# AlwinEsch/pvr.rtl.radiofm

Measured on AMD Instinct MI355X. Metric: IQ MS/s demodulated (whole node) + achieved HBM GB/s on FIR stage, higher is better.
Workload: dtype f32

## Files before the change

pvr.rtl.radiofm_amd/csrc/fmd_k_serial.hip.h:

```cpp
#pragma once

#include "fmd_k_common.hip.h"

namespace fmd
{


#ifndef FMD_DS
#define FMD_DS 32
#endif
constexpr int DS = FMD_DS;
static_assert(DS == 32 || DS == 16, "chunk size");
typedef float fmd_v4f __attribute__((ext_vector_type(4)));
constexpr int STAGE_RS = 65;
constexpr unsigned FM_UNROLL = 4;

template <int NG, bool EXCL, bool MIX = true>
__global__ __launch_bounds__(128 * NG) void k_demod_serial(
    const float2* __restrict__ demod, unsigned Mstride, unsigned M, unsigned C, unsigned CP,
    DemodConsts k, ChannelState st, float2* __restrict__ br, unsigned Hbb,
    float2* __restrict__ mix, unsigned Hmix, const double* __restrict__ sctab_g, FmdSincosTab sct,
    unsigned stereo_q, long long* __restrict__ wg_probe, float osc_after_re, float osc_after_im)
{
  const long long probe_r0 = wg_probe ? (long long)__builtin_amdgcn_s_memrealtime() : 0;
  const long long probe_c0 = wg_probe ? (long long)__builtin_readcyclecounter() : 0;
  __shared__ float chunk_all[NG][2][DS][64];
  __shared__ float2 stage_all[NG][2][DS][STAGE_RS];
  constexpr unsigned SCTAB_N = FMD_SINCOS_P256_SIZE;
  __shared__ __attribute__((aligned(1024))) double sctab[2 * SCTAB_N];
  __shared__ __attribute__((aligned(512))) float atab[FMD_ATAN_TAB_FLOATS];
  constexpr bool PAIRSYNC = NG > 1;
  __shared__ unsigned done_all[NG][2];
  if (threadIdx.x < 2 * NG)
    (&done_all[0][0])[threadIdx.x] = 0;
  __builtin_amdgcn_s_setprio(3);
  if (EXCL)
    asm volatile("" ::: "v255", "a255");
  for (unsigned i = threadIdx.x; i < 2 * SCTAB_N; i += 128 * NG)
    sctab[i] = sctab_g[i];
  if (threadIdx.x == 0)
    fmd_atan_table_fill(atab);
  const unsigned lane = threadIdx.x & 63u;
  const unsigned wave = threadIdx.x >> 6;
  const unsigned role = wave & 1u;
  const unsigned grp = wave >> 1;
  float (*chunk)[DS][64] = chunk_all[grp];
  float2 (*stage)[DS][STAGE_RS] = stage_all[grp];
  const unsigned done_fm = (unsigned)(size_t)&done_all[grp][0];
  const unsigned done_2nd = (unsigned)(size_t)&done_all[grp][1];
  double m16 = -1.0 / 6.0;
  asm volatile("" : "+v"(m16));
  const unsigned c0 = (blockIdx.x * NG + grp) * 64 + lane;
  const bool active = c0 < C;
  const unsigned c = active ? c0 : C - 1;
  const unsigned nchunks = (M + DS - 1) / DS;
  const float2* __restrict__ row = demod + (size_t)c * Mstride;
  for (unsigned u = role; u < DS; u += 2)
    stage[0][u][lane] = row[min(u, M - 1)];
  __syncthreads();

  if (role == 0)
  {
    float nco_phase = st.F(F_NCO_PHASE)[c], nco_incr = st.F(F_NCO_INCR)[c];
    __builtin_amdgcn_s_waitcnt(0);
    for (unsigned j = 0; j <= nchunks; j++)
    {
      if (PAIRSYNC)
      {
        if (j == nchunks)
          break;
        lds_wait_ge(done_2nd, j, st.spin_limit, st.err);
      }
      if (j < nchunks)
      {
        const unsigned m0 = j * DS;
        const unsigned cnt = min((unsigned)DS, M - m0);
        auto fm_sample = [&](unsigned u) -> uint32_t {
          const float2 sin_ = stage[j & 1][u][lane];
          const float sre = sin_.x, sim = sin_.y;
          float sn, cs;
          fmd_sincos_p256_finish(fmd_sincos_p256_lookup_lds(nco_phase, sctab), m16, &sn, &cs);
          const fmd_v2f dd = fmd_pk_add_cross((fmd_v2f){sre, sim} * cs, (fmd_v2f){sre, sim} * sn);
          const float dre = dd.x, dim = dd.y;
          uint32_t lit;
          const float err = -fmd_atan2f_tab_core(dim, dre, atab, &lit);
          const fmd_v2f ba = (fmd_v2f){k.pll_beta, k.pll_alpha} * err;
          nco_incr += ba.x;
          nco_incr = fminf(fmaxf(nco_incr, k.nco_ll), k.nco_hl);
          nco_phase += nco_incr + ba.y;
          {
            const uint32_t pb = fmd_f2u(nco_phase);
            uint32_t khi = (~pb & 0x80000000u) | 0x401921fbu;
            khi = pb < 0x40c90fdbu ? 0u : khi;
            const uint64_t kb = ((uint64_t)khi << 32) | 0x54442d18u;
            double off;
            memcpy(&off, &kb, 8);
            nco_phase = (float)((double)nco_phase + off);
          }
          chunk[j & 1][u][lane] = nco_incr;
          return lit;
        };
        auto fm_sample_literal = [&](unsigned u) {
          const float2 sin_ = stage[j & 1][u][lane];
          float sn, cs;
          fmd_sincos_p256k(nco_phase, sctab, m16, &sn, &cs);
          const fmd_v2f dd = fmd_pk_add_cross((fmd_v2f){sin_.x, sin_.y} * cs, (fmd_v2f){sin_.x, sin_.y} * sn);
          const float e2 = -fmd_atan2f(dd.y, dd.x);
          float in2 = nco_incr + k.pll_beta * e2;
          in2 = (in2 < k.nco_ll) ? k.nco_ll : in2;
          in2 = (in2 > k.nco_hl) ? k.nco_hl : in2;
          float ph2 = nco_phase + (in2 + k.pll_alpha * e2);
          const double pd2 = (double)ph2;
          if (pd2 >= FMD_K_2PI)
            ph2 = (float)fmod(pd2, FMD_K_2PI);
          while (ph2 < 0)
            ph2 = (float)((double)ph2 + FMD_K_2PI);
          nco_incr = in2;
          nco_phase = ph2;
          chunk[j & 1][u][lane] = nco_incr;
        };
#ifdef FMD_DBG_NO_FM
        if (true)
        {
          for (unsigned u = 0; u < cnt; u++)
            chunk[j & 1][u][lane] = nco_incr;
        }
        else
#endif
        if (cnt == (unsigned)DS)
        {
#pragma unroll 1
          for (unsigned u = 0; u < (unsigned)DS; u += FM_UNROLL)
          {
            const float phase_g = nco_phase, incr_g = nco_incr;
            uint32_t worst = 0;
#pragma unroll
            for (unsigned v = 0; v < FM_UNROLL; v++)
              worst = max(worst, fm_sample(u + v));
            if (__builtin_expect(FMD_ANY_LANE(worst >= FMD_ATAN_RARE_LIMIT), 0))
            {
              nco_phase = phase_g;
              nco_incr = incr_g;
#pragma unroll 1
              for (unsigned v = 0; v < FM_UNROLL; v++)
                fm_sample_literal(u + v);
            }
          }
        }
        else
        {
#pragma unroll 1
          for (unsigned u = 0; u < cnt; u++)
          {
            const float phase_g = nco_phase, incr_g = nco_incr;
            if (__builtin_expect(FMD_ANY_LANE(fm_sample(u) >= FMD_ATAN_RARE_LIMIT), 0))
            {
              nco_phase = phase_g;
              nco_incr = incr_g;
              fm_sample_literal(u);
            }
          }
        }
      }
      if (PAIRSYNC)
        lds_publish(done_fm, j + 1);
      else
        lds_barrier();
    }
    if (active)
    {
      st.F(F_NCO_PHASE)[c] = nco_phase;
      st.F(F_NCO_INCR)[c] = nco_incr;
    }
  }
  else
  {
    float p_i1 = st.F(F_P_I1)[c], p_i2 = st.F(F_P_I2)[c], p_q1 = st.F(F_P_Q1)[c], p_q2 = st.F(F_P_Q2)[c];
    float p_x1 = st.F(F_P_X1)[c], p_freq = st.F(F_P_FREQ)[c], p_phase = st.F(F_P_PHASE)[c];
    float p_level = 1000.0f;
    float o_re = st.F(F_OSC_RE)[c], o_im = st.F(F_OSC_IM)[c];
    float dc = st.F(F_DC_OFF)[c];
    __builtin_amdgcn_s_waitcnt(0);
    FmdSincosP256 p_sc = fmd_sincos_p256_lookup_lds(p_phase, sctab);
    float vsum = 0.0f, vsumsq = 0.0f;
    char* __restrict__ br_rows = reinterpret_cast<char*>(br + (size_t)Hbb * CP);
    char* __restrict__ mix_rows = reinterpret_cast<char*>(mix + (size_t)Hmix * CP);
    unsigned row_off = c * (unsigned)sizeof(float2);
    const unsigned row_step = CP * (unsigned)sizeof(float2);
    constexpr unsigned CO_LPR = DS / 2;
    constexpr unsigned CO_RPI = 64 / CO_LPR;
    const unsigned co_row = lane / CO_LPR, co_col = lane % CO_LPR;
    unsigned co_off[DS / 2];
#pragma unroll
    for (unsigned i = 0; i < DS / 2; i++)
      co_off[i] = min((blockIdx.x * NG + grp) * 64 + CO_RPI * i + co_row, C - 1) *
                      (Mstride * (unsigned)sizeof(float2)) +
                  co_col * 16u;
    for (unsigned j = 0; j <= nchunks; j++)
    {
      const unsigned pf0 = (j + 1) * DS;
      const bool staging = (j + 1) < nchunks;
      fmd_v4f pre_c[DS / 2];
      if (staging)
      {
        const float2* sb = demod + pf0;
#pragma unroll
        for (unsigned i = 0; i < DS / 2; i += 4)
          asm volatile("global_load_dwordx4 %0, %4, %8\n\t"
                       "global_load_dwordx4 %1, %5, %8\n\t"
                       "global_load_dwordx4 %2, %6, %8\n\t"
                       "global_load_dwordx4 %3, %7, %8"
                       : "=&v"(pre_c[i]), "=&v"(pre_c[i + 1]), "=&v"(pre_c[i + 2]), "=&v"(pre_c[i + 3])
                       : "v"(co_off[i]), "v"(co_off[i + 1]), "v"(co_off[i + 2]), "v"(co_off[i + 3]), "s"(sb)
                       : "memory");
      }
      unsigned stores_behind = 0;
      if (PAIRSYNC && j >= 1)
        lds_wait_ge(done_fm, j, st.spin_limit, st.err);
      if (j >= 1)
      {
        const unsigned m0 = (j - 1) * DS;
        const unsigned cnt = min((unsigned)DS, M - m0);
        float pinc_next = chunk[(j - 1) & 1][0][lane];
        auto second_sample = [&](unsigned u) {
            const float pinc = 2 * pinc_next;
            pinc_next = chunk[(j - 1) & 1][min(u + 1, (unsigned)DS - 1)][lane];
            dc = (float)((1 - 0.0001) * (double)dc + 0.0001 * (double)pinc);
            const float v = (pinc - dc) * k.demod_gain;
            vsum += v;
            vsumsq += v * v;
            float ps, pc;
            fmd_sincos_p256_finish(p_sc, m16, &ps, &pc);
            const float tone = 2 * ps * pc;
            float ph_i = ps * v;
            float ph_q = pc * v;
            ph_i = k.p_b0 * ph_i - k.p_a1 * p_i1 - k.p_a2 * p_i2;
            ph_q = k.p_b0 * ph_q - k.p_a1 * p_q1 - k.p_a2 * p_q2;
            p_i2 = p_i1;
            p_i1 = ph_i;
            p_q2 = p_q1;
            p_q1 = ph_q;
            const float ratio = ph_q / ph_i;
            const float sgn = (ph_q > 0) ? 1.0f : -1.0f;
            const float perr = (ph_i > fabsf(ph_q)) ? ratio : sgn;
            p_level = (ph_i < p_level) ? ph_i : p_level;
            p_freq += k.p_lf_b0 * perr + k.p_lf_b1 * p_x1;
            p_x1 = perr;
            p_freq = fmaxf(k.p_minfreq, fminf(k.p_maxfreq, p_freq));
            p_phase += p_freq;
            {
              const double pd = (double)p_phase;
              const float down = (float)(pd - FMD_K_2PI);
              p_phase = (pd > FMD_K_2PI) ? down : p_phase;
            }
            p_sc = fmd_sincos_p256_lookup_lds(p_phase, sctab);
            __builtin_amdgcn_sched_barrier(0);
            if constexpr (MIX)
            {
            float2 osc;
            osc.x = o_re * k.osc_cos - o_im * k.osc_sin;
            osc.y = o_im * k.osc_cos + o_re * k.osc_sin;
            const float gn = (float)(1.95 - (double)(o_re * o_re + o_im * o_im));
            o_re = gn * osc.x;
            o_im = gn * osc.y;
            const float zero = 0.0f;
#ifdef FMD_DBG_NO_STORES
            vsum += tone * (2 * v) + ((v * osc.x) - (zero * osc.y)) + ((v * osc.y) + (zero * osc.x));
#else
            *reinterpret_cast<float2*>(br_rows + row_off) = make_float2(v, tone * (2 * v));
            *reinterpret_cast<float2*>(mix_rows + row_off) =
                make_float2((v * osc.x) - (zero * osc.y), (v * osc.y) + (zero * osc.x));
#endif
            }
            else
              *reinterpret_cast<float2*>(br_rows + row_off) = make_float2(v, tone * (2 * v));
            row_off += row_step;
        };
#ifdef FMD_DBG_NO_2ND
        if (true)
        {
        }
        else
#endif
        if (cnt == (unsigned)DS)
        {
#pragma unroll 1
          for (unsigned u = 0; u < (unsigned)DS; u += 2)
          {
            second_sample(u);
            second_sample(u + 1);
          }
        }
        else
        {
#pragma unroll 1
          for (unsigned u = 0; u < cnt; u++)
            second_sample(u);
        }
        stores_behind = (MIX ? 2 : 1) * cnt;
      }
      if (staging)
      {
        if (stores_behind >= (MIX ? 2 : 1) * DS)
        {
          if ((MIX ? 2 : 1) * DS == 64)
            asm volatile("s_waitcnt vmcnt(63)" ::: "memory");
          else if ((MIX ? 2 : 1) * DS == 32)
            asm volatile("s_waitcnt vmcnt(31)" ::: "memory");
          else
            asm volatile("s_waitcnt vmcnt(15)" ::: "memory");
        }
        else
          asm volatile("s_waitcnt vmcnt(0)" ::: "memory");
#pragma unroll
        for (unsigned i = 0; i < DS / 2; i++)
        {
          stage[(j + 1) & 1][2 * co_col][CO_RPI * i + co_row] = make_float2(pre_c[i].x, pre_c[i].y);
          stage[(j + 1) & 1][2 * co_col + 1][CO_RPI * i + co_row] = make_float2(pre_c[i].z, pre_c[i].w);
        }
      }
      if (PAIRSYNC)
        lds_publish(done_2nd, j + 1);
      else
        lds_barrier();
    }
    if (active)
    {
      st.F(F_P_I1)[c] = p_i1;
      st.F(F_P_I2)[c] = p_i2;
      st.F(F_P_Q1)[c] = p_q1;
      st.F(F_P_Q2)[c] = p_q2;
      st.F(F_P_X1)[c] = p_x1;
      st.F(F_P_FREQ)[c] = p_freq;
      st.F(F_P_PHASE)[c] = p_phase;
      st.F(F_P_LEVEL)[c] = p_level;
      st.F(F_OSC_RE)[c] = MIX ? o_re : osc_after_re;
      st.F(F_OSC_IM)[c] = MIX ? o_im : osc_after_im;
      st.F(F_DC_OFF)[c] = dc;
      {
        int cnt = st.I(I_P_LOCK_CNT)[c];
        if (2 * p_level > k.p_minsignal)
        {
          if (cnt < k.p_lock_delay)
            cnt += (int)M;
        }
        else
          cnt = 0;
        st.I(I_P_LOCK_CNT)[c] = cnt;
        st.I(I_STEREO)[c] = cnt >= k.p_lock_delay;
        st.I(I_STEREO_Q0 + (int)stereo_q)[c] = cnt >= k.p_lock_delay;
      }
      {
        const float mean = vsum / (float)M;
        const float rms = sqrtf(vsumsq / (float)M);
        st.F(F_BB_MEAN)[c] = 0.95f * st.F(F_BB_MEAN)[c] + 0.05f * mean;
        st.F(F_BB_LEVEL)[c] = 0.95f * st.F(F_BB_LEVEL)[c] + 0.05f * rms;
      }
    }
  }
  if (wg_probe && threadIdx.x == 64)
  {
    wg_probe[3 * blockIdx.x] = probe_r0;
    wg_probe[3 * blockIdx.x + 1] = (long long)__builtin_amdgcn_s_memrealtime();
    const unsigned hw_id = __builtin_amdgcn_s_getreg((31 << 11) | 4);
    const unsigned xcc_id = __builtin_amdgcn_s_getreg((31 << 11) | 20);
    wg_probe[3 * blockIdx.x + 2] = (((long long)__builtin_readcyclecounter() - probe_c0) & 0xffffffffffll) |
                                   ((long long)((hw_id >> 8) & 0xffu) << 40) |
                                   ((long long)(xcc_id & 0xfu) << 48);
  }
}

}
```

pvr.rtl.radiofm_amd/csrc/fmd_math.h:

```cpp
#ifndef FMD_MATH_H
#define FMD_MATH_H

#include <math.h>
#include <stdint.h>
#include <string.h>
#ifndef __cplusplus
#include <stdbool.h>
#endif

#ifdef __HIPCC__
#define FMD_HD __host__ __device__ static inline
#define FMD_HD_NOINLINE __host__ __device__ static __attribute__((noinline))
#else
#define FMD_HD static inline
#define FMD_HD_NOINLINE static __attribute__((noinline))
#endif

#if defined(__clang__)
typedef float fmd_v2f __attribute__((ext_vector_type(2)));
#else
typedef float fmd_v2f __attribute__((vector_size(8)));
#endif

FMD_HD fmd_v2f fmd_pk_add_cross(fmd_v2f a, fmd_v2f b)
{
#if defined(__HIP_DEVICE_COMPILE__)
  fmd_v2f r;
  asm("v_pk_add_f32 %0, %1, %2 op_sel:[0,1] op_sel_hi:[1,0] neg_lo:[0,1]" : "=v"(r) : "v"(a), "v"(b));
  return r;
#else
  fmd_v2f r = {a[0] - b[1], a[1] + b[0]};
  return r;
#endif
}

#define FMD_K_2PI (2.0 * 3.14159265358979323846)
#define FMD_K_PI (3.14159265358979323846)
#define FMD_K_PI2 (FMD_K_PI / 2.0)

#if defined(__HIP_DEVICE_COMPILE__)
#define FMD_ANY_LANE(cond) (__builtin_amdgcn_ballot_w64(cond) != 0)
#else
#define FMD_ANY_LANE(cond) (cond)
#endif

FMD_HD float fmd_div_midrange(float n, float d)
{
#if defined(__HIP_DEVICE_COMPILE__)
  const float r0 = __builtin_amdgcn_rcpf(d);
  const float e0 = __builtin_fmaf(-d, r0, 1.0f);
  const float r1 = __builtin_fmaf(e0, r0, r0);
  const float q0 = n * r1;
  const float e1 = __builtin_fmaf(-d, q0, n);
  const float q1 = __builtin_fmaf(e1, r1, q0);
  const float e2 = __builtin_fmaf(-d, q1, n);
  return __builtin_fmaf(e2, r1, q1);
#else
  return n / d;
#endif
}

FMD_HD uint32_t fmd_f2u(float f)
{
  uint32_t u;
  memcpy(&u, &f, 4);
  return u;
}
FMD_HD float fmd_u2f(uint32_t u)
{
  float f;
  memcpy(&f, &u, 4);
  return f;
}

FMD_HD float fmd_u8_to_f32(unsigned b)
{
  const float f = (float)b;
  const float s = __builtin_fmaf(f, 0x1.01p-7f, -1.0f);
  return __builtin_fmaf(f, 0x1.010102p-23f, s);
}

FMD_HD float fmd_s8_to_f32(int v)
{
  return (float)v * 0x1p-7f;
}
FMD_HD float fmd_s16_to_f32(int v)
{
  return (float)v * 0x1p-15f;
}

FMD_HD float fmd_ciq16_to_f32(int v)
{
  return (float)v * 0x1p-13f;
}

FMD_HD int fmd_f32_to_s16_count(float x, unsigned* clipped)
{
  const float y = x * 32768.0f;
  if (y != y)
    return 0;
  const float r = rintf(y);
  *clipped += (r > 32767.0f) | (r < -32768.0f);
  return (int)fminf(fmaxf(r, -32768.0f), 32767.0f);
}
FMD_HD int fmd_f32_to_s16(float x)
{
  unsigned clipped = 0;
  return fmd_f32_to_s16_count(x, &clipped);
}

FMD_HD int fmd_f32_to_mpx16(float x)
{
  const float y = x * 8192.0f;
  if (y != y)
    return 0;
  return (int)fminf(fmaxf(rintf(y), -32768.0f), 32767.0f);
}

FMD_HD float fmd_atanf(float x)
{
  const float atanhi0 = 4.6364760399e-01f, atanhi1 = 7.8539812565e-01f,
              atanhi2 = 9.8279368877e-01f, atanhi3 = 1.5707962513e+00f;
  const float atanlo0 = 5.0121582440e-09f, atanlo1 = 3.7748947079e-08f,
              atanlo2 = 3.4473217170e-08f, atanlo3 = 7.5497894159e-08f;
  const float aT0 = 3.3333334327e-01f, aT1 = -2.0000000298e-01f, aT2 = 1.4285714924e-01f,
              aT3 = -1.1111110449e-01f, aT4 = 9.0908870101e-02f, aT5 = -7.6918758452e-02f,
              aT6 = 6.6610731184e-02f, aT7 = -5.8335702866e-02f, aT8 = 4.9768779427e-02f,
              aT9 = -3.6531571299e-02f, aT10 = 1.6285819933e-02f;
  const float one = 1.0f;
  float w, s1, s2, z;
  int32_t hx = (int32_t)fmd_f2u(x);
  int32_t ix = hx & 0x7fffffff;
  int id;
  float hi = 0.0f, lo = 0.0f;
  if (ix >= 0x4c000000)
  {
    if (ix > 0x7f800000)
      return x + x;
    if (hx > 0)
      return atanhi3 + atanlo3;
    return -atanhi3 - atanlo3;
  }
  if (ix < 0x3ee00000)
  {
    if (ix < 0x31000000)
      return x;
    id = -1;
  }
  else
  {
    x = fabsf(x);
    if (ix < 0x3f980000)
    {
      if (ix < 0x3f300000)
      {
        id = 0;
        x = (2.0f * x - one) / (2.0f + x);
        hi = atanhi0;
        lo = atanlo0;
      }
      else
      {
        id = 1;
        x = (x - one) / (x + one);
        hi = atanhi1;
        lo = atanlo1;
      }
    }
    else
    {
      if (ix < 0x401c0000)
      {
        id = 2;
        x = (x - 1.5f) / (one + 1.5f * x);
        hi = atanhi2;
        lo = atanlo2;
      }
      else
      {
        id = 3;
        x = -1.0f / x;
        hi = atanhi3;
        lo = atanlo3;
      }
    }
  }
  z = x * x;
  w = z * z;
  s1 = z * (aT0 + w * (aT2 + w * (aT4 + w * (aT6 + w * (aT8 + w * aT10)))));
  s2 = w * (aT1 + w * (aT3 + w * (aT5 + w * (aT7 + w * aT9))));
  if (id < 0)
    return x - x * (s1 + s2);
  z = hi - ((x * (s1 + s2) - lo) - x);
  return (hx < 0) ? -z : z;
}

FMD_HD_NOINLINE float fmd_atan2f(float y, float x)
{
  const float tiny = 1.0e-30f, pi_o_4 = 7.8539818525e-01f, pi_o_2 = 1.5707963705e+00f,
              pi = 3.1415927410e+00f, pi_lo = -8.7422776573e-08f;
  float z;
  int32_t hx = (int32_t)fmd_f2u(x), hy = (int32_t)fmd_f2u(y);
  int32_t ix = hx & 0x7fffffff, iy = hy & 0x7fffffff;
  if ((ix > 0x7f800000) || (iy > 0x7f800000))
    return x + y;
  if (hx == 0x3f800000)
    return fmd_atanf(y);
  int m = ((hy >> 31) & 1) | ((hx >> 30) & 2);
  if (iy == 0)
  {
    switch (m)
    {
      case 0:
      case 1:
        return y;
      case 2:
        return pi + tiny;
      default:
        return -pi - tiny;
    }
  }
  if (ix == 0)
    return (hy < 0) ? -pi_o_2 - tiny : pi_o_2 + tiny;
  if (ix == 0x7f800000)
  {
    if (iy == 0x7f800000)
    {
      switch (m)
      {
        case 0:
          return pi_o_4 + tiny;
        case 1:
          return -pi_o_4 - tiny;
        case 2:
          return 3.0f * pi_o_4 + tiny;
        default:
          return -3.0f * pi_o_4 - tiny;
      }
    }
    else
    {
      switch (m)
      {
        case 0:
          return 0.0f;
        case 1:
          return -0.0f;
        case 2:
          return pi + tiny;
        default:
          return -pi - tiny;
      }
    }
  }
  if (iy == 0x7f800000)
    return (hy < 0) ? -pi_o_2 - tiny : pi_o_2 + tiny;
  int32_t k = (iy - ix) >> 23;
  if (k > 60)
    z = pi_o_2 + 0.5f * pi_lo;
  else if (hx < 0 && k < -60)
    z = 0.0f;
  else
    z = fmd_atanf(fabsf(y / x));
  switch (m)
  {
    case 0:
      return z;
    case 1:
      return fmd_u2f(fmd_f2u(z) ^ 0x80000000u);
    case 2:
      return pi - (z - pi_lo);
    default:
      return (z - pi_lo) - pi;
  }
}

FMD_HD void fmd_sincos_nco(float phase, float* s, float* c)
{
  const double x = (double)phase;
  const double k = __builtin_rint(x * 6.36619772367581382433e-01);
  double r = __builtin_fma(-k, 1.57079632673412561417e+00, x);
  r = __builtin_fma(-k, 6.07710050650619224932e-11, r);
  const double z = r * r;
  double ps = __builtin_fma(z, 1.58969099521155010221e-10, -2.50507602534068634195e-08);
  ps = __builtin_fma(z, ps, 2.75573137070700676789e-06);
  ps = __builtin_fma(z, ps, -1.98412698298579493134e-04);
  ps = __builtin_fma(z, ps, 8.33333333332248946124e-03);
  ps = __builtin_fma(z, ps, -1.66666666666666324348e-01);
  const double sr = __builtin_fma(r * z, ps, r);
  double pc = __builtin_fma(z, -1.13596475577881948265e-11, 2.08757232129817482790e-09);
  pc = __builtin_fma(z, pc, -2.75573143513906633035e-07);
  pc = __builtin_fma(z, pc, 2.48015872894767294178e-05);
  pc = __builtin_fma(z, pc, -1.38888888888741095749e-03);
  pc = __builtin_fma(z, pc, 4.16666666666666019037e-02);
  const double hz = 0.5 * z;
  const double w = 1.0 - hz;
  const double cr = w + (((1.0 - w) - hz) + z * z * pc);
  const int n = (int)k;
  double so = (n & 1) ? cr : sr;
  double co = (n & 1) ? sr : cr;
  so = (n & 2) ? -so : so;
  co = ((n + 1) & 2) ? -co : co;
  *s = (float)so;
  *c = (float)co;
}

#define FMD_ATAN_TAB_FLOATS 40
FMD_HD void fmd_atan_table_fill(float* t)
{
  const float v[5][8] = {
      {1.0f, 0.0f, 0.0f, 1.0f, 0.0f, 0.0f, 0, 0},
      {2.0f, -1.0f, 1.0f, 2.0f, 4.6364760399e-01f, 5.0121582440e-09f, 0, 0},
      {1.0f, -1.0f, 1.0f, 1.0f, 7.8539812565e-01f, 3.7748947079e-08f, 0, 0},
      {1.0f, -1.5f, 1.5f, 1.0f, 9.8279368877e-01f, 3.4473217170e-08f, 0, 0},
      {0.0f, -1.0f, 1.0f, 0.0f, 1.5707962513e+00f, 7.5497894159e-08f, 0, 0}};
  for (int r = 0; r < 5; r++)
    for (int k = 0; k < 8; k++)
      t[r * 8 + k] = v[r][k];
}

#if defined(__HIP_DEVICE_COMPILE__)
FMD_HD unsigned long long fmd_pack2f(float lo, float hi)
{
  return (unsigned long long)fmd_f2u(lo) | ((unsigned long long)fmd_f2u(hi) << 32);
}
#endif

#define FMD_ATAN_RARE_LIMIT (0x4c000000u - 0x31000000u)
FMD_HD float fmd_atan2f_tab_core(float y, float x, const float* tab, uint32_t* rare_measure)
{
  const float aT0 = 3.3333334327e-01f, aT1 = -2.0000000298e-01f, aT2 = 1.4285714924e-01f,
              aT3 = -1.1111110449e-01f, aT4 = 9.0908870101e-02f, aT5 = -7.6918758452e-02f,
              aT6 = 6.6610731184e-02f, aT7 = -5.8335702866e-02f, aT8 = 4.9768779427e-02f,
              aT9 = -3.6531571299e-02f, aT10 = 1.6285819933e-02f;
  const float pi = 3.1415927410e+00f, pi_lo = -8.7422776573e-08f;
  const float q = fabsf(y / x);
  const uint32_t iq = fmd_f2u(q);
  const uint32_t rare_m = iq - 0x31000000u;
  const uint32_t ic = iq;
  const float qc = fmd_u2f(ic);
  const int r = 4 + ((int32_t)(ic - 0x3ee00000u) >> 31) + ((int32_t)(ic - 0x3f300000u) >> 31) +
                ((int32_t)(ic - 0x3f980000u) >> 31) + ((int32_t)(ic - 0x401c0000u) >> 31);
  const float* t = tab + 8 * r;
#if defined(__HIP_DEVICE_COMPILE__)
  const float a2 = (float)__builtin_amdgcn_ubfe(0x02242u, 4u * (unsigned)r, 4u);
  const float c2 = (float)__builtin_amdgcn_ubfe(0x23220u, 4u * (unsigned)r, 4u);
#else
  const float a2 = (float)((0x02242u >> (4u * (unsigned)r)) & 0xfu);
  const float c2 = (float)((0x23220u >> (4u * (unsigned)r)) & 0xfu);
#endif
  const fmd_v2f ac = {a2, c2};
  const fmd_v2f nd = fmd_pk_add_cross(ac * qc, ac);
  const float num = nd[0];
  const float den = nd[1];
  const float xr = fmd_div_midrange(num, den);
  const float z = xr * xr;
  const float w = z * z;
  const fmd_v2f wz = {w, z};
  fmd_v2f hc;
#if defined(__HIP_DEVICE_COMPILE__)
  asm("v_pk_mul_f32 %0, %1, %2 op_sel_hi:[0,1]\n\t"
      "v_pk_add_f32 %0, %0, %3\n\t"
      "v_pk_mul_f32 %0, %0, %1 op_sel_hi:[1,0]\n\t"
      "v_pk_add_f32 %0, %0, %4\n\t"
      "v_pk_mul_f32 %0, %0, %1 op_sel_hi:[1,0]\n\t"
      "v_pk_add_f32 %0, %0, %5\n\t"
      "v_pk_mul_f32 %0, %0, %1 op_sel_hi:[1,0]\n\t"
      "v_pk_add_f32 %0, %0, %6\n\t"
      "v_pk_mul_f32 %0, %0, %1 op_sel_hi:[1,0]\n\t"
      "v_pk_add_f32 %0, %0, %7\n\t"
      "v_pk_mul_f32 %0, %0, %1"
      : "=&v"(hc)
      : "v"(wz), "s"(fmd_pack2f(0.0f, aT10)), "s"(fmd_pack2f(aT9, aT8)), "s"(fmd_pack2f(aT7, aT6)),
        "s"(fmd_pack2f(aT5, aT4)), "s"(fmd_pack2f(aT3, aT2)), "s"(fmd_pack2f(aT1, aT0)));
#else
  hc = (fmd_v2f){0.0f, aT10} * w + (fmd_v2f){aT9, aT8};
  hc = hc * w + (fmd_v2f){aT7, aT6};
  hc = hc * w + (fmd_v2f){aT5, aT4};
  hc = hc * w + (fmd_v2f){aT3, aT2};
  hc = hc * w + (fmd_v2f){aT1, aT0};
  hc = hc * wz;
#endif
  const float p = xr * (hc[1] + hc[0]);
  const float at = t[4] - ((p - t[5]) - xr);
  const float left = pi - (at - pi_lo);
  const float base = ((int32_t)fmd_f2u(x) < 0) ? left : at;
  *rare_measure = rare_m;
  return fmd_u2f(fmd_f2u(base) ^ (fmd_f2u(y) & 0x80000000u));
}

FMD_HD float fmd_atan2f_tab(float y, float x, const float* tab)
{
  uint32_t rare_m;
  float res = fmd_atan2f_tab_core(y, x, tab, &rare_m);
  const bool rare = rare_m >= FMD_ATAN_RARE_LIMIT;
  if (FMD_ANY_LANE(rare))
  {
    if (rare)
      res = fmd_atan2f(y, x);
  }
  return res;
}

struct FmdSincosTab
{
  double inv_h, h_hi, h_lo;
};
#define FMD_SINCOS_TAB_SIZE 1024
FMD_HD void fmd_sincos_tab(float phase, const double* tab , struct FmdSincosTab t,
                           float* s, float* c)
{
  const double x = (double)phase;
  const double magic = 6755399441055744.0;
  const double tt = __builtin_fma(x, t.inv_h, magic);
  const double kf = tt - magic;
  uint64_t ttu;
  memcpy(&ttu, &tt, 8);
  const int k = (int)(uint32_t)ttu;
  double r = __builtin_fma(-kf, t.h_hi, x);
  r = __builtin_fma(-kf, t.h_lo, r);
  const double S = tab[2 * (k & (FMD_SINCOS_TAB_SIZE - 1))];
  const double C = tab[2 * (k & (FMD_SINCOS_TAB_SIZE - 1)) + 1];
  const double r2 = r * r;
  const double sr = __builtin_fma(r * r2, __builtin_fma(r2, 1.0 / 120.0, -1.0 / 6.0), r);
  const double cm1 = r2 * __builtin_fma(r2, 1.0 / 24.0, -0.5);
  const double so = S + __builtin_fma(C, sr, S * cm1);
  const double co = C + __builtin_fma(-S, sr, C * cm1);
  *s = (float)so;
  *c = (float)co;
}

FMD_HD double fmd_fma_const(double x, double a, double b)
{
#if defined(__HIP_DEVICE_COMPILE__)
  double r;
  asm("v_fma_f64 %0, %1, %2, %3" : "=v"(r) : "v"(x), "s"(a), "v"(b));
  return r;
#else
  return __builtin_fma(x, a, b);
#endif
}

#define FMD_SINCOS_P256_SIZE 2048
struct FmdSincosP256
{
  double S, C;
  float r;
};
FMD_HD struct FmdSincosP256 fmd_sincos_p256_lookup(float phase, const double* tab )
{
  const float big = 49152.0f;
  const float t = phase + big;
  const uint32_t k = fmd_f2u(t) & (FMD_SINCOS_P256_SIZE - 1);
  const float kx = t - big;
  struct FmdSincosP256 e;
  e.r = phase - kx;
  e.S = tab[2 * k];
  e.C = tab[2 * k + 1];
  return e;
}
FMD_HD struct FmdSincosP256 fmd_sincos_p256_lookup_lds(float phase, const double* tab)
{
  const float big = 32768.0f;
  const float t = phase + big;
  uint32_t off;
#if defined(__HIP_DEVICE_COMPILE__)
  asm("v_mul_u32_u24 %0, %1, 16" : "=v"(off) : "v"(t));
#else
  off = (fmd_f2u(t) & 0xffffffu) * 16u;
#endif
  const float kx = t - big;
  struct FmdSincosP256 e;
  e.r = phase - kx;
  typedef double fmd_v2d_ __attribute__((vector_size(16)));
  const fmd_v2d_ sc = *(const fmd_v2d_*)((const char*)tab + off);
  e.S = sc[0];
  e.C = sc[1];
  return e;
}
FMD_HD void fmd_sincos_p256_finish(struct FmdSincosP256 e, double m16, float* s, float* c)
{
  const double r = (double)e.r, S = e.S, C = e.C;
  const double r2 = r * r;
#if defined(__HIP_DEVICE_COMPILE__)
  double sr, st;
  asm("v_fma_f64 %1, %2, %3, %4\n\t"
      "v_fma_f64 %0, %5, %1, %6"
      : "=&v"(sr), "=&v"(st)
      : "v"(r2), "s"(1.0 / 120.0), "v"(m16), "v"(r * r2), "v"(r));
#else
  const double sr = __builtin_fma(r * r2, fmd_fma_const(r2, 1.0 / 120.0, m16), r);
#endif
  const double cm1 = r2 * __builtin_fma(r2, 1.0 / 24.0, -0.5);
  const double so = S + __builtin_fma(C, sr, S * cm1);
  const double co = C + __builtin_fma(-S, sr, C * cm1);
  *s = (float)so;
  *c = (float)co;
}
FMD_HD void fmd_sincos_p256k(float phase, const double* tab , double m16, float* s, float* c)
{
  fmd_sincos_p256_finish(fmd_sincos_p256_lookup(phase, tab), m16, s, c);
}
FMD_HD void fmd_sincos_p256(float phase, const double* tab , float* s, float* c)
{
  fmd_sincos_p256k(phase, tab, -1.0 / 6.0, s, c);
}

FMD_HD float fmd_rds_arctan2(float y, float x)
{
  if (x == 0.0f)
  {
    if (y > 0.0f)
      return (float)FMD_K_PI2;
    if (y == 0.0f)
      return 0.0f;
    return (float)-FMD_K_PI2;
  }
  float angle;
  float z = y / x;
  if (fabsf(z) < 1.0f)
  {
    angle = (float)((double)z / (1.0 + 0.2854 * (double)z * (double)z));
    if (x < 0.0f)
    {
      if (y < 0.0f)
        return (float)((double)angle - FMD_K_PI);
      return (float)((double)angle + FMD_K_PI);
    }
  }
  else
  {
    angle = (float)(FMD_K_PI2 - (double)z / ((double)(z * z) + 0.2854));
    if (y < 0.0f)
      return (float)((double)angle - FMD_K_PI);
  }
  return angle;
}

#endif
```

Baseline: 301,200.

## Unroll FM loop by eight, branchless phase wraps and cheaper atan range indexing

Doubles the FM PLL inner unroll from 4 to 8 samples per rare-check group and folds the rare measures in pairs. It replaces the double-precision phase-wrap offset construction with unsigned-min based wraps for both the FM NCO and the pilot PLL. It also replaces the four-compare atan range index with a popcount-based index and a 64-bit packed coefficient lookup. The goal is fewer ALU ops on the serial PLL critical path, at the cost of more register pressure and a larger rollback window when a rare atan case triggers.

```diff
diff --git a/pvr.rtl.radiofm_amd/csrc/fmd_k_serial.hip.h b/pvr.rtl.radiofm_amd/csrc/fmd_k_serial.hip.h
--- a/pvr.rtl.radiofm_amd/csrc/fmd_k_serial.hip.h
+++ b/pvr.rtl.radiofm_amd/csrc/fmd_k_serial.hip.h
@@ -13,7 +13,11 @@
 static_assert(DS == 32 || DS == 16, "chunk size");
 typedef float fmd_v4f __attribute__((ext_vector_type(4)));
 constexpr int STAGE_RS = 65;
-constexpr unsigned FM_UNROLL = 4;
+#ifndef FMD_FM_UNROLL
+#define FMD_FM_UNROLL 8
+#endif
+constexpr unsigned FM_UNROLL = FMD_FM_UNROLL;
+static_assert(FM_UNROLL % 2 == 0 && DS % FM_UNROLL == 0, "the group's rare measures are folded in pairs");
 
 template <int NG, bool EXCL, bool MIX = true>
 __global__ __launch_bounds__(128 * NG) void k_demod_serial(
@@ -89,13 +93,7 @@
           nco_incr = fminf(fmaxf(nco_incr, k.nco_ll), k.nco_hl);
           nco_phase += nco_incr + ba.y;
           {
-            const uint32_t pb = fmd_f2u(nco_phase);
-            uint32_t khi = (~pb & 0x80000000u) | 0x401921fbu;
-            khi = pb < 0x40c90fdbu ? 0u : khi;
-            const uint64_t kb = ((uint64_t)khi << 32) | 0x54442d18u;
-            double off;
-            memcpy(&off, &kb, 8);
-            nco_phase = (float)((double)nco_phase + off);
+            nco_phase = fmd_wrap_0_2pi(nco_phase);
           }
           chunk[j & 1][u][lane] = nco_incr;
           return lit;
@@ -135,8 +133,11 @@
             const float phase_g = nco_phase, incr_g = nco_incr;
             uint32_t worst = 0;
 #pragma unroll
-            for (unsigned v = 0; v < FM_UNROLL; v++)
-              worst = max(worst, fm_sample(u + v));
+            for (unsigned v = 0; v < FM_UNROLL; v += 2)
+            {
+              const uint32_t lit0 = fm_sample(u + v), lit1 = fm_sample(u + v + 1);
+              worst = max(max(worst, lit0), lit1);
+            }
             if (__builtin_expect(FMD_ANY_LANE(worst >= FMD_ATAN_RARE_LIMIT), 0))
             {
               nco_phase = phase_g;
@@ -249,9 +250,7 @@
             p_freq = fmaxf(k.p_minfreq, fminf(k.p_maxfreq, p_freq));
             p_phase += p_freq;
             {
-              const double pd = (double)p_phase;
-              const float down = (float)(pd - FMD_K_2PI);
-              p_phase = (pd > FMD_K_2PI) ? down : p_phase;
+              p_phase = fmd_wrap_above_2pi(p_phase);
             }
             p_sc = fmd_sincos_p256_lookup_lds(p_phase, sctab);
             __builtin_amdgcn_sched_barrier(0);
diff --git a/pvr.rtl.radiofm_amd/csrc/fmd_math.h b/pvr.rtl.radiofm_amd/csrc/fmd_math.h
--- a/pvr.rtl.radiofm_amd/csrc/fmd_math.h
+++ b/pvr.rtl.radiofm_amd/csrc/fmd_math.h
@@ -71,6 +71,22 @@
   float f;
   memcpy(&f, &u, 4);
   return f;
+}
+
+FMD_HD float fmd_wrap_above_2pi(float phase)
+{
+  const float down = (float)((double)phase - FMD_K_2PI);
+  const uint32_t a = fmd_f2u(down), b = fmd_f2u(phase);
+  return fmd_u2f(a < b ? a : b);
+}
+
+FMD_HD float fmd_wrap_0_2pi(float phase)
+{
+  const double pd = (double)phase;
+  const uint32_t down = fmd_f2u((float)(pd - FMD_K_2PI)), up = fmd_f2u((float)(pd + FMD_K_2PI));
+  const uint32_t b = fmd_f2u(phase);
+  const uint32_t m = down < b ? down : b;
+  return fmd_u2f(up < m ? up : m);
 }
 
 FMD_HD float fmd_u8_to_f32(unsigned b)
@@ -326,6 +342,23 @@
 }
 #endif
 
+FMD_HD uint32_t fmd_atan_range_index(uint32_t iq)
+{
+  const int32_t below = 0x7f3 - (int32_t)(iq >> 19);
+  const int32_t s = below < 0 ? 0 : (below > 24 ? 24 : below);
+  const uint32_t last = (uint32_t)((int32_t)(iq - 0x401c0000u) >> 31);
+  return (uint32_t)__builtin_popcount(0x80802001u >> s) + last;
+}
+FMD_HD void fmd_atan_range_ac2(uint32_t r, float* a2, float* c2)
+{
+  uint64_t w = 0x0202040203020200ull >> (8u * r);
+#if defined(__HIP_DEVICE_COMPILE__)
+  asm("" : "+v"(w));
+#endif
+  *c2 = (float)(uint32_t)(w & 0xffu);
+  *a2 = (float)(uint32_t)((w >> 32) & 0xffu);
+}
+
 #define FMD_ATAN_RARE_LIMIT (0x4c000000u - 0x31000000u)
 FMD_HD float fmd_atan2f_tab_core(float y, float x, const float* tab, uint32_t* rare_measure)
 {
@@ -339,16 +372,10 @@
   const uint32_t rare_m = iq - 0x31000000u;
   const uint32_t ic = iq;
   const float qc = fmd_u2f(ic);
-  const int r = 4 + ((int32_t)(ic - 0x3ee00000u) >> 31) + ((int32_t)(ic - 0x3f300000u) >> 31) +
-                ((int32_t)(ic - 0x3f980000u) >> 31) + ((int32_t)(ic - 0x401c0000u) >> 31);
+  const uint32_t r = fmd_atan_range_index(ic);
   const float* t = tab + 8 * r;
-#if defined(__HIP_DEVICE_COMPILE__)
-  const float a2 = (float)__builtin_amdgcn_ubfe(0x02242u, 4u * (unsigned)r, 4u);
-  const float c2 = (float)__builtin_amdgcn_ubfe(0x23220u, 4u * (unsigned)r, 4u);
-#else
-  const float a2 = (float)((0x02242u >> (4u * (unsigned)r)) & 0xfu);
-  const float c2 = (float)((0x23220u >> (4u * (unsigned)r)) & 0xfu);
-#endif
+  float a2, c2;
+  fmd_atan_range_ac2(r, &a2, &c2);
   const fmd_v2f ac = {a2, c2};
   const fmd_v2f nd = fmd_pk_add_cross(ac * qc, ac);
   const float num = nd[0];
```

Result: no change. 303,200 (median of 4 runs) (+0.7%).
